# felrock/PyRacecarSimulator

Hardware: AMD Instinct MI355X
Metric: million rays/sec, 1081-beam scans (higher is better)
Workload: dtype f32

## Files before the change

pyracecarsimulator_amd/csrc/abi_fan.hip:

```cpp
#include "abi_internal.h"
#include "scan_kernels.h"
#include "crash_kernels.h"
#include "pf_kernels.h"
#include "mcl_kernels.h"
#include "launch_plan.h"

#include <array>
#include <utility>

static_assert(plan::WG == scan::WG && plan::STREAM_HDR == scan::STREAM_HDR && plan::STRIPE_BINS == scan::STRIPE_BINS &&
                  plan::STRIPE_MAX_PER_LANE == scan::STRIPE_MAX_PER_LANE && plan::DRAIN_CAP == scan::DRAIN_CAP &&
                  plan::DRAIN_FIELDS == scan::DRAIN_FIELDS && plan::INLINE_REC_BYTES == (int)sizeof(scan::BlockRec),
              "launch_plan.h and rm_kernels.h disagree about the stream kernels' LDS layout");

extern "C" int rl_method_create(rl_map *m, int kind, float max_range_px, int theta_disc,
                                rl_method **out)
{
    if (!m || !out) return fail(RL_ERR_INVALID, "rl_method_create: null pointer");
    if (!(max_range_px > 0.0f)) return fail(RL_ERR_INVALID, "max_range_px must be > 0");
    if (kind < RL_BRESENHAM || kind > RL_GIANT_LUT)
        return fail(RL_ERR_INVALID, "unknown range method kind %d", kind);
    if ((kind == RL_CDDT || kind == RL_GIANT_LUT) && (theta_disc < 2 || theta_disc > 65536))
        return fail(RL_ERR_INVALID, "theta_disc must be in [2, 65536] for CDDT / GiantLUT (got %d)",
                    theta_disc);
// ... 786 lines not shown
{
    rl_method *h = L.h;
    const int form = plan::cddt_theta_form(L.pl);
    if (form < 0) return fail(RL_ERR_INVALID, "internal: plan names an uninstantiated kernel (%s)", L.pl.name);
    const bool fused = form == plan::CDDT_THETA_FUSED;
    int rc;
    if ((rc = ensure_cddt(h, L.stream))) return rc;
    const size_t prep_bytes = (((size_t)L.n_poses * 16) + 255) & ~(size_t)255;
    if ((rc = L.cx->cddt_r.ensure(prep_bytes + (fused ? 0 : (size_t)h->cdp.theta_disc * (size_t)L.n_poses * sizeof(float)))))
        return rc;
    float4 *d_prep = (float4 *)L.cx->cddt_r.p;
    float *d_r = (float *)((char *)L.cx->cddt_r.p + prep_bytes);
    if (L.timing == 2) HIPCHK(hipEventRecord(h->ev0, L.stream));
    hipLaunchKernelGGL(cddt_theta_prep_kernel, dim3((unsigned)std::max(1, std::min((L.n_poses + 255) / 256, L.m->n_cu * 8))),
                       dim3(256), 0, L.stream, L.m->mp, L.f, h->cdp, L.d_poses, d_prep);
    if (fused) {
        hipLaunchKernelGGL(cddt_theta_fused_kernel, L.grid, L.block, L.lds, L.stream, L.m->mp, L.f, h->cdp, L.d_poses,
                           (const float4 *)d_prep, L.d_out, L.pl.nl);
        return RL_OK;
    }
    if (form == plan::CDDT_THETA_SEARCH2)
        hipLaunchKernelGGL(cddt_theta_search2_kernel, L.grid, L.block, 0, L.stream, L.m->mp, L.f, h->cdp, L.d_poses,
                           (const float4 *)d_prep, d_r, L.pl.bands);
    else
        hipLaunchKernelGGL(cddt_theta_search_kernel, L.grid, L.block, 0, L.stream, L.m->mp, L.f, h->cdp, L.d_poses,
                           (const float4 *)d_prep, d_r, L.pl.bands);
    const int n_grp = (L.n_poses + (1 << L.pl.ch) - 1) >> L.pl.ch;
    hipLaunchKernelGGL(cddt_theta_fan_kernel, dim3((unsigned)std::max(1, std::min(n_grp, L.m->n_cu * 8))), L.block, L.lds,
                       L.stream, L.m->mp, L.f, h->cdp, L.d_poses, (const float *)d_r, L.d_out, L.pl.ch, L.pl.nl);
    return RL_OK;
}

static int launch_cddt_rays(const FanLaunch &L)
{
    int rc;
    if ((rc = ensure_cddt(L.h, L.stream))) return rc;
    if (L.timing == 2) HIPCHK(hipEventRecord(L.h->ev0, L.stream));
    hipLaunchKernelGGL(cddt_fan_kernel, L.grid, L.block, 0, L.stream, L.m->mp, L.f, L.h->cdp, L.d_poses, L.d_out);
    return RL_OK;
}

static int launch_bl_stream(const FanLaunch &L)
{
    rl_method *h = L.h;
    int rc;
    if ((rc = ensure_blpad(h, L.stream))) return rc;
    if ((rc = bin_poses(h, *L.cx, L.d_poses, L.n_poses, 1, L.stream, L.pl.binning))) return rc;
    StreamParams sp{};
    sp.rec = (const PoseRec *)L.cx->rec_sorted.p;
    sp.order = (const uint32_t *)L.cx->order.p;
    sp.div_B = make_fastdiv((uint32_t)L.num_rays);
    sp.low_water = h->opt.low_water >= 0 ? h->opt.low_water : 12;
    sp.n_bands = L.pl.bands;
    sp.plain_store = L.plain_store;
    if (L.timing == 2) HIPCHK(hipEventRecord(h->ev0, L.stream));
    if (L.aux)
        hipLaunchKernelGGL((bl_fan_stream_kernel<true, 1024>), L.grid, L.block, L.lds, L.stream, L.m->mp, L.f, sp, h->blp,
                           L.d_out, L.d_hits, L.d_steps);
    else
        hipLaunchKernelGGL((bl_fan_stream_kernel<false, 1024>), L.grid, L.block, L.lds, L.stream, L.m->mp, L.f, sp, h->blp,
                           L.d_out, L.d_hits, L.d_steps);
    return RL_OK;
}

static int launch_bl_lds(const FanLaunch &L)
{
    size_t lds_bl = 0;
    BlParams bp = make_bl(L.h, L.num_rays, lds_bl);
    const bool bl = L.pl.kernel == RL_K_BL_LDS;
    if (lds_bl > 48 * 1024) {
        const void *fa = bl ? reinterpret_cast<const void *>(&bl_fan_kernel<true>)
                            : reinterpret_cast<const void *>(&occ_fan_lds_kernel<true>);
        const void *fb = bl ? reinterpret_cast<const void *>(&bl_fan_kernel<false>)
                            : reinterpret_cast<const void *>(&occ_fan_lds_kernel<false>);
        HIPCHK(hipFuncSetAttribute(fa, hipFuncAttributeMaxDynamicSharedMemorySize, (int)lds_bl));
        HIPCHK(hipFuncSetAttribute(fb, hipFuncAttributeMaxDynamicSharedMemorySize, (int)lds_bl));
    }
    if (L.timing == 2) HIPCHK(hipEventRecord(L.h->ev0, L.stream));
#define LAUNCH_BL(K) hipLaunchKernelGGL((K), L.grid, L.block, lds_bl, L.stream, L.m->mp, L.f, bp, L.d_poses, L.d_out, L.d_hits, L.d_steps)
    if (bl) { if (L.aux) LAUNCH_BL(bl_fan_kernel<true>); else LAUNCH_BL(bl_fan_kernel<false>); }
    else    { if (L.aux) LAUNCH_BL(occ_fan_lds_kernel<true>); else LAUNCH_BL(occ_fan_lds_kernel<false>); }
#undef LAUNCH_BL
    return RL_OK;
}

static int launch_rm_literal(const FanLaunch &L)
{
    const LiteralParams lt = make_literal(L.m);
    const long n_rays = (long)L.n_poses * L.num_rays;
    if (L.timing == 2) HIPCHK(hipEventRecord(L.h->ev0, L.stream));
    if (L.aux)
        hipLaunchKernelGGL((rm_literal_kernel<true, false>), L.grid, L.block, 0, L.stream, L.m->mp, L.f, lt, L.d_poses, n_rays,
                           L.d_out, L.d_hits, L.d_steps);
    else
        hipLaunchKernelGGL((rm_literal_kernel<false, false>), L.grid, L.block, 0, L.stream, L.m->mp, L.f, lt, L.d_poses, n_rays,
                           L.d_out, L.d_hits, L.d_steps);
    return RL_OK;
}

static int launch_rm_chunk(const FanLaunch &L)
{
    CrashParams cp{nullptr, 0.0, nullptr, 1};
    if (L.crash) cp = *L.crash;
    if (L.timing == 2) HIPCHK(hipEventRecord(L.h->ev0, L.stream));
#define LAUNCH_CHUNK(A, C) hipLaunchKernelGGL((rm_fan_kernel<A, C>), L.grid, L.block, L.lds, L.stream, L.m->mp, L.f, L.d_poses, \
                                              L.d_out, L.d_hits, L.d_steps, cp)
    if (L.crash) { if (L.aux) LAUNCH_CHUNK(true, true); else LAUNCH_CHUNK(false, true); }
    else         { if (L.aux) LAUNCH_CHUNK(true, false); else LAUNCH_CHUNK(false, false); }
#undef LAUNCH_CHUNK
    return RL_OK;
}

static int launch_rm_stream_family(const FanLaunch &L)
{
    rl_method *h = L.h;
    const rl_launch_plan &pl = L.pl;
    int rc;
    CrashParams cp{nullptr, 0.0, nullptr, 1};
    if (L.crash) cp = *L.crash;
    if ((rc = L.cx->rec.ensure((size_t)L.n_poses * sizeof(PoseRec)))) return rc;
    if ((rc = L.cx->order.ensure((size_t)L.n_poses * sizeof(uint32_t)))) return rc;
    if ((rc = L.cx->keys.ensure((size_t)L.n_poses * sizeof(uint32_t)))) return rc;
    if ((rc = ensure_step_map(h, L.stream))) return rc;
    if (pl.binning != RL_BIN_NONE &&
        (rc = bin_poses(h, *L.cx, L.d_poses, L.n_poses, 0, L.stream, pl.binning)))
        return rc;
    PadMap pm{};
    pm.pdt = (const float *)((const char *)h->pdt.p + h->pdt_base_off);
    pm.stride = h->pstride;
    pm.nstride = (int)h->pdt_mask;
    pm.pad = h->pad;
    pm.k4 = h->pdt_k4;
    pm.div_stride = make_fastdiv((uint32_t)h->pstride);
    pm.res = L.m->res;
    if (pl.code) {
        if (h->code_n <= 0 || pl.code_entries != h->code_n)
            return fail(RL_ERR_INVALID, "internal: code-map plan (%d entries) without a matching palette (%d)", pl.code_entries, h->code_n);
        pm.pdt = (const float *)((const char *)h->cmap.p + h->cbase_off);
        pm.stride = h->cstride;
        pm.nstride = (int)h->cmask;
        pm.k4 = h->ck4;
    }
    StreamParams sp{};
    sp.code_tab = (const float *)h->ctab.p;
    sp.code_n = pl.code ? h->code_n : 0;
    sp.tail_g1 = pl.gen1 > 0 ? pl.gen1 / std::max(pl.bands, 1) : 0;
    sp.tail_pct = std::min(h->opt.tail_pct, h->opt.tail_wg_pct);
    sp.rec = (const PoseRec *)L.cx->rec_sorted.p;
    sp.order = (const uint32_t *)L.cx->order.p;
    sp.d0 = (const float *)L.cx->d0.p;
    if ((rc = ensure_fan_table(h, L.f, L.fov, L.stream, &sp.fan_tab))) return rc;
    sp.div_B = make_fastdiv((uint32_t)L.num_rays);
    sp.low_water = h->opt.low_water >= 0 ? h->opt.low_water : ((pl.record_source != 0 && pl.slots >= 2) ? 20 : 12);
    sp.n_bands = pl.bands;
    sp.raw_poses = L.d_poses;
    sp.map = L.m->d_mp;
    sp.k_max = pl.k_max;
    sp.cpp = (uint32_t)((L.num_rays + 63) / 64);
    sp.div_cpp = make_fastdiv(sp.cpp);
    sp.drain_prio = h->drain_prio;
    sp.spec_drain = h->spec_drain;
    sp.spec_stretch = h->spec_stretch;
    sp.drain_cap = h->drain_cap;
    sp.drain_stretch = h->drain_stretch;
    sp.group_drain = h->group_drain;
    if (pl.kernel == RL_K_RM_STREAM_LIT) sp.lit = make_literal(L.m);
    sp.plain_store = L.plain_store;
    sp.dbg = nullptr;
    const int waves_per_wg = pl.block / 64;
    if (h->opt.debug_stamps) {
        if ((rc = L.cx->dbg.ensure((size_t)pl.grid * waves_per_wg * 4 * sizeof(uint64_t)))) return rc;
        sp.dbg = (unsigned long long *)L.cx->dbg.p;
        h->last_dbg = L.cx->dbg.p;
    }
    sp.stripe = pl.record_source == 2 ? 1 : pl.record_source == 3 ? 2 : 0;
    sp.run_log2 = pl.run_log2;
    h->last_grid = pl.grid * waves_per_wg / WAVES_PER_WG;
    const bool handoff = h->handoff && pl.slots >= 2 && pl.tiled && h->spec_drain > 0 && !h->opt.debug_stamps &&
                         pl.kernel == RL_K_RM_STREAM && !pl.code;
    int cap_log2 = 4;
    const int n_src = pl.grid * waves_per_wg;
    if (handoff) {
        cap_log2 = h->handoff_cap >= 64 ? 6 : (h->handoff_cap >= 32 ? 5 : (h->handoff_cap >= 16 ? 4 : 3));
        if ((rc = L.cx->left_rec.ensure(((size_t)n_src << cap_log2) * sizeof(LeftoverRec)))) return rc;
        if ((rc = L.cx->left_cnt.ensure((size_t)n_src * sizeof(uint32_t)))) return rc;
        sp.left_rec = (LeftoverRec *)L.cx->left_rec.p;
        sp.left_cnt = (uint32_t *)L.cx->left_cnt.p;
        sp.left_cap_log2 = cap_log2;
        sp.drain_cap = std::min(sp.drain_cap, 1 << cap_log2);
    }
    if (L.timing == 2) HIPCHK(hipEventRecord(h->ev0, L.stream));
    if ((rc = dispatch_rm_stream(pl, L.stream, pm, L.f, sp, L.d_out, L.d_hits, L.d_steps, cp))) return rc;
    if (handoff) {
        const int lw = h->handoff_wg / 64;
        const int n_lw = (n_src + (64 >> cap_log2) - 1) / (64 >> cap_log2);
        const dim3 lgrid((unsigned)((n_lw + lw - 1) / lw)), lblock((unsigned)h->handoff_wg);
        if (L.crash)
            hipLaunchKernelGGL((rm_leftover_kernel<true>), lgrid, lblock, 0, L.stream, pm, L.f, (const LeftoverRec *)sp.left_rec,
                               (const uint32_t *)sp.left_cnt, n_src, cap_log2, h->drain_stretch, sp.plain_store, L.d_out, cp);
        else
            hipLaunchKernelGGL((rm_leftover_kernel<false>), lgrid, lblock, 0, L.stream, pm, L.f, (const LeftoverRec *)sp.left_rec,
                               (const uint32_t *)sp.left_cnt, n_src, cap_log2, h->drain_stretch, sp.plain_store, L.d_out, cp);
    }
    return RL_OK;
}

FanCall FanCall::slice(int p0, int np, CrashParams *marks) const
{
    const size_t r0 = (size_t)p0 * num_rays;
// ... 889 lines not shown
```

pyracecarsimulator_amd/csrc/abi_internal.h:

```cpp
#pragma once
#pragma GCC visibility push(default)
#include "../../include/scanlib.h"
#pragma GCC visibility pop
#include "scan_params.h"
#include "literal_math.h"

#include <hip/hip_runtime.h>

#include <algorithm>
#include <climits>
#include <cmath>
#include <cstdarg>
#include <cstdio>
#include <cstring>
#include <atomic>
#include <condition_variable>
#include <functional>
#include <memory>
#include <mutex>
#include <shared_mutex>
#include <new>
#include <string>
#include <thread>
#include <type_traits>
// ... 141 lines not shown
        const int rc = b.ensure(n);
        return rc ? rc : up((T *)b, host, n);
    }
    template <class T>
    int fill(DevPtr<T> &b, int byte, size_t n)
    {
        const int rc = b.ensure(n);
        if (rc) return rc;
        HIPCHK(hipMemsetAsync((T *)b, byte, n * sizeof(T), st));
        return RL_OK;
    }
    template <class T>
    int zero(DevPtr<T> &b, size_t n)
    {
        return fill(b, 0, n);
    }
    template <class T>
    int down(T *host_or_null, const T *dev, size_t n)
    {
        if (host_or_null) HIPCHK(hipMemcpyAsync(host_or_null, dev, n * sizeof(T), hipMemcpyDeviceToHost, st));
        return RL_OK;
    }
    template <class T>
    int down(T *host_or_null, const DevPtr<T> &dev, size_t n)
    {
        return down(host_or_null, (const T *)dev, n);
    }
    int finish()
    {
        finished = true;
        HIPCHK(hipStreamSynchronize(st));
        return RL_OK;
    }
};

struct rl_map {
    std::vector<rl_map *> reps;
    int device = 0;
    int clock_khz = 0;
    int rows = 0, cols = 0;
    float res = 0, ox = 0, oy = 0, oyaw = 0;
    DevPtr<uint8_t> d_occ;
    DevPtr<uint8_t> d_occ_base;
    DevPtr<int32_t> d_stamp;
    Pinned<int32_t> pin_stamp;
    int stamp_cap = 0, n_stamped = 0;
    DevPtr<int> d_g;
    DevPtr<float> d_dt;
    DevPtr<uint32_t> d_bits;
    int bits_stride = 0;
    Stream stream;
    std::atomic<uint64_t> epoch{0};
    MapParams mp{};
    DevPtr<MapParams> d_mp;
    bool want_edges = false;
    DevPtr<uint32_t> d_edges, d_n_edges;
    Pinned<uint32_t> pin_n_edges;
    uint32_t n_edges = 0;
    int n_cu = 256;
    std::mutex mu;
    std::shared_mutex tables_mu;
    std::shared_mutex multi_mu;
    std::atomic<bool> broken{false};
};

struct LaunchCtx {
    hipStream_t stream = nullptr;
    bool bound = false;
    uint64_t last_use = 0;
    DevBuf rec, rec_sorted, order, keys, hist, pose_first, dbg, d0, cddt_r;
    DevBuf left_rec, left_cnt;
    DevBuf pf_r;
    int crash_epoch = 0;
};
constexpr int N_LAUNCH_CTX = 8;

struct TableDep {
    Event ev;
    hipStream_t built_on = nullptr;
    bool pending = false;
};


struct MultiPool {
    struct Worker {
        std::thread th;
        std::mutex mu;
        std::condition_variable cv;
        const std::function<int()> *job = nullptr;
        bool has = false, done = false, stop = false;
        int rc = 0;
        std::string err;
        int device = 0;
    };
    std::vector<std::unique_ptr<Worker>> w;

    void start(const std::vector<int> &devices)
    {
        for (size_t i = 1; i < devices.size(); ++i) {
            auto wk = std::make_unique<Worker>();
            wk->device = devices[i];
            Worker *raw = wk.get();
            wk->th = std::thread([raw]() {
                (void)hipSetDevice(raw->device);
                std::unique_lock<std::mutex> lk(raw->mu);
                for (;;) {
                    raw->cv.wait(lk, [raw]() { return raw->has || raw->stop; });
// ... 242 lines not shown
```

pyracecarsimulator_amd/csrc/abi_map.hip:

```cpp
#include "abi_internal.h"
#include "edt_kernels.h"

static thread_local std::string g_err = "";

int fail(int code, const char *fmt, ...)
{
    char buf[512];
    va_list ap;
    va_start(ap, fmt);
    vsnprintf(buf, sizeof buf, fmt, ap);
    va_end(ap);
    g_err = buf;
    return code;
}

int fail_map_broken() { return fail(RL_ERR_INVALID, "multi-device map is inconsistent after a failed update: destroy it"); }
const std::string &last_error() { return g_err; }
void set_last_error(const std::string &msg) { g_err = msg; }

extern "C" const char *rl_last_error(void) { return g_err.c_str(); }
extern "C" const char *rl_version(void) { return "scanlib-amd 0.6 (gfx950)"; }

extern "C" int rl_device_count(void)
{
// ... 131 lines not shown
    if (m->want_edges) m->n_edges = *m->pin_n_edges;
    return RL_OK;
}

extern "C" int rl_map_create(const uint8_t *occ, int rows, int cols, float res, float ox,
                             float oy, float oyaw, int device, rl_map **out)
{
    if (!occ || !out) return fail(RL_ERR_INVALID, "rl_map_create: null pointer");
    if (rows <= 0 || cols <= 0 || rows > 16384 || cols > 16384)
        return fail(RL_ERR_INVALID, "rl_map_create: rows/cols must be in [1,16384] (got %dx%d)",
                    rows, cols);
    if (!(res > 0.0f)) return fail(RL_ERR_INVALID, "rl_map_create: resolution must be > 0");
    int rc = check_device(device);
    if (rc) return rc;
    std::unique_ptr<rl_map, decltype(&rl_map_destroy)> own(new (std::nothrow) rl_map(), rl_map_destroy);
    rl_map *m = own.get();
    if (!m) return fail(RL_ERR_NOMEM, "out of host memory");
    m->device = device;
    m->rows = rows;
    m->cols = cols;
    m->res = res;
    m->ox = ox;
    m->oy = oy;
    m->oyaw = oyaw;
    m->bits_stride = (cols + 31) / 32;
    if (hipSetDevice(device) != hipSuccess) return fail(RL_ERR_HIP, "hipSetDevice failed");
    hipDeviceProp_t prop;
    if (hipGetDeviceProperties(&prop, device) == hipSuccess) {
        m->n_cu = prop.multiProcessorCount;
        m->clock_khz = prop.clockRate;
    }
    const size_t n = (size_t)rows * cols;
    if (m->stream.create() != hipSuccess || m->d_occ.alloc(n) || m->d_g.alloc(n * sizeof(int)) ||
        m->d_dt.alloc(n * sizeof(float)) || m->d_bits.alloc((size_t)rows * m->bits_stride * sizeof(uint32_t)))
        return fail(RL_ERR_NOMEM, "device allocation for a %dx%d map failed", rows, cols);
    if (hipMemcpyAsync(m->d_occ, occ, n, hipMemcpyHostToDevice, m->stream) != hipSuccess)
        return fail(RL_ERR_HIP, "map upload failed");
    if ((rc = map_build_tables(m))) return rc;

    MapParams &p = m->mp;
    p.dt = m->d_dt;
    p.bits = m->d_bits;
    p.bits_stride = m->bits_stride;
    p.rows = rows;
    p.cols = cols;
    p.frows = (float)rows;
    p.fcols = (float)cols;
    p.res = res;
    p.inv_res = (float)(1.0 / (double)res);
    p.ox = ox;
    p.oy = oy;
    p.wa = -oyaw;
    host_sincosf(p.wa, p.wa_sin, p.wa_cos);
    if (m->d_mp.alloc(sizeof(MapParams)) || hipMemcpy(m->d_mp, &m->mp, sizeof(MapParams), hipMemcpyHostToDevice) != hipSuccess)
        return fail(RL_ERR_NOMEM, "map parameter upload failed");
    *out = own.release();
    return RL_OK;
}

extern "C" int rl_map_create_multi(const uint8_t *occ, int rows, int cols, float res, float ox, float oy,
                                   float oyaw, const int *devices, int n_devices, rl_map **out)
{
    if (!occ || !out || !devices) return fail(RL_ERR_INVALID, "rl_map_create_multi: null pointer");
    if (n_devices < 1 || n_devices > 64) return fail(RL_ERR_INVALID, "rl_map_create_multi: 1..64 devices (got %d)", n_devices);
    std::unique_ptr<rl_map, decltype(&rl_map_destroy)> own(new (std::nothrow) rl_map(), rl_map_destroy);
    rl_map *m = own.get();
    if (!m) return fail(RL_ERR_NOMEM, "out of host memory");
    for (int i = 0; i < n_devices; ++i) {
        rl_map *r = nullptr;
        const int rc = rl_map_create(occ, rows, cols, res, ox, oy, oyaw, devices[i], &r);
        if (rc) {
            const std::string keep = g_err;
            own.reset();
            g_err = keep;
            return rc;
        }
        m->reps.push_back(r);
    }
    const rl_map *r0 = m->reps[0];
    m->device = r0->device;
    m->rows = rows;
    m->cols = cols;
    m->res = res;
    m->ox = ox;
    m->oy = oy;
    m->oyaw = oyaw;
    m->n_cu = r0->n_cu;
    m->clock_khz = r0->clock_khz;
    m->mp = r0->mp;
    *out = own.release();
    return RL_OK;
}

extern "C" int rl_map_n_devices(const rl_map *m) { return m ? (m->reps.empty() ? 1 : (int)m->reps.size()) : 0; }

extern "C" rl_map *rl_map_replica(rl_map *m, int i)
{
    if (!m) return nullptr;
    if (m->reps.empty()) return i == 0 ? m : nullptr;
    return (i >= 0 && i < (int)m->reps.size()) ? m->reps[i] : nullptr;
}

extern "C" int rl_map_update(rl_map *m, const uint8_t *occ)
{
    if (!m || !occ) return fail(RL_ERR_INVALID, "rl_map_update: null pointer");
    if (!m->reps.empty()) {
        std::lock_guard<std::mutex> lk(m->mu);
        std::unique_lock<std::shared_mutex> wl(m->multi_mu);
// ... 122 lines not shown
```

pyracecarsimulator_amd/csrc/rm_kernels.h:

```cpp
#pragma once
#include "scan_device.h"
#include "scan_params.h"
#include "literal_math.h"

namespace scan {

constexpr int WG = 256;
constexpr int WAVES_PER_WG = WG / 64;

struct CrashParams {
    const double *edge;
    double thresh;
    int *first_crashed;
    int group;
    int mark;
};

__device__ __forceinline__ void crash_note(const CrashParams &cp, uint32_t pose)
{
    if (cp.group == 0) {
        cp.first_crashed[pose] = cp.mark;
        return;
    }
    int *slot = &cp.first_crashed[pose / (uint32_t)cp.group];
// ... 173 lines not shown
    for (uint32_t i = lo; i < hi; ++i) {
        const float d = val[i];
        if (d > 0.0f) {
            idx[i] = k;
            if (k < cap) tab[k] = __builtin_fmaxf(d * coeff, 1.0f);
            ++k;
        }
    }
    if (tid == 0) {
        if (total + 2u <= cap) {
            tab[total] = PDT_HIT;
            tab[total + 1] = PDT_OUTSIDE;
        }
        n_out[0] = total + 2u;
        n_out[1] = total + 2u <= cap ? 0u : 1u;
    }
}

template <int ES>
__global__ __launch_bounds__(256) void pad_code_tiled_kernel(const float *__restrict__ dt, int rows, int cols,
                                                             void *__restrict__ cmap, TiledGeom tg, float coeff,
                                                             float max_range, const uint32_t *__restrict__ idx,
                                                             uint32_t nb, const uint32_t *__restrict__ n_pal)
{
    const uint32_t n_free = n_pal[0] - 2u;
    const int pr = blockIdx.y;
    const int r = pr - tg.padr;
    for (int pc = blockIdx.x * blockDim.x + threadIdx.x; pc < tg.pcols; pc += gridDim.x * blockDim.x) {
        const int c = pc - tg.pad;
        uint32_t code = n_free + 1u;
        if (r >= 0 && r < rows && c >= 0 && c < cols) {
            const float d = dt[(size_t)r * cols + c];
            if (d <= 0.0f) {
                code = n_free;
            } else if (__builtin_fmaxf(d * coeff, 1.0f) < max_range) {
                const uint32_t d2 = (uint32_t)__builtin_fmaf(d, d, 0.5f);
                code = d2 < nb ? idx[d2] : n_free + 1u;
            }
        }
        char *at = reinterpret_cast<char *>(cmap) + code_tiled_byte(pr, pc, tg.K, ES);
        if (ES == 1) *reinterpret_cast<uint16_t *>(at) = (uint16_t)(code << 2);
        else *reinterpret_cast<uint8_t *>(at) = (uint8_t)code;
    }
}

#define PDT_NO_RAY 2.5e38f
__device__ __forceinline__ float pose_first_step(const MapParams &m, float gx, float gy, uint32_t flags,
                                                 float coeff)
{
    if (flags & POSE_INVALID) return PDT_NO_RAY;
    const float v = m.dt[(size_t)(int)gy * m.cols + (int)gx];
    return v <= 0.0f ? 0.0f : __builtin_fmaxf(v * coeff, 1.0f);
}

__device__ __forceinline__ uint32_t tile_key(int ty, int tx, int tiles_xs, int n_tiles)
{
    const int tiles_x = tiles_xs & 0xffff, rps = tiles_xs >> 16;
    if (rps == 0) return (uint32_t)(ty * tiles_x + tx);
    const int tiles_y = n_tiles / tiles_x;
    const int y0 = (ty / rps) * rps, h = min(rps, tiles_y - y0);
    return (uint32_t)(y0 * tiles_x + tx * h + (ty - y0));
}

__device__ __forceinline__ uint32_t pose_record(const MapParams &m, const float *__restrict__ poses,
                                                int p, int tile_shift, int tiles_x, int n_tiles,
                                                PoseRec &r, bool walk_outside = false)
{
    float thg;
    world_to_grid(m, poses[3 * (size_t)p], poses[3 * (size_t)p + 1], poses[3 * (size_t)p + 2], r.gx,
                  r.gy, thg);
    det_sincosf(thg, r.st, r.ct);
    const bool fin = (r.ct - r.ct) + (r.st - r.st) == 0.0f;
    const bool inb = r.gx > -1.0f && r.gx < m.fcols && r.gy > -1.0f && r.gy < m.frows;
    if (walk_outside) {
        const bool sane = fin && __builtin_fabsf(r.gx) < 1e9f && __builtin_fabsf(r.gy) < 1e9f;
        if (!sane) {
            r.gx = 0.0f; r.gy = 0.0f; r.ct = 1.0f; r.st = 0.0f;
            return ((uint32_t)n_tiles - 1) | POSE_INVALID;
        }
        if (!inb) return (uint32_t)n_tiles - 1;
    } else if (!(fin && inb)) {
        r.gx = 0.0f; r.gy = 0.0f; r.ct = 1.0f; r.st = 0.0f;
        return ((uint32_t)n_tiles - 1) | POSE_INVALID;
    }
    return tile_key((int)r.gy >> tile_shift, (int)r.gx >> tile_shift, tiles_x, n_tiles);
}

__device__ __forceinline__ uint32_t pose_record_lit(const MapParams &m, const LiteralParams &lp, const float *__restrict__ poses,
                                                    int p, PoseRec &r)
{
    const float xw = poses[3 * (size_t)p], yw = poses[3 * (size_t)p + 1], thw = poses[3 * (size_t)p + 2];
    float x = (xw - m.ox) * m.inv_res;
    float y = (yw - m.oy) * m.inv_res;
    const float temp = x;
    x = lp.wcos * x - lp.wsin * y;
    y = lp.wsin * temp + lp.wcos * y;
    r.gx = x;
    r.gy = y;
    r.ct = thw;
    r.st = 0.0f;
    const bool fin = (thw - thw) == 0.0f;
    const bool inb = x > -1.0f && x < m.fcols && y > -1.0f && y < m.frows;
    if (!(fin && inb)) {
        r.gx = 0.0f; r.gy = 0.0f; r.ct = 0.0f;
        return POSE_INVALID;
    }
    return 0u;
}

__global__ __launch_bounds__(1024) void pose_bin_kernel(MapParams m, const float *__restrict__ poses,
                                                        int n, PoseRec *__restrict__ rec,
                                                        PoseRec *__restrict__ rec_sorted,
                                                        uint32_t *__restrict__ order,
                                                        uint32_t *__restrict__ keys, int tile_shift,
                                                        int tiles_x, int n_tiles, int do_sort, int walk_outside,
                                                        float *__restrict__ d0, float coeff)
{
    extern __shared__ uint32_t hist[];
    uint32_t *part = hist + n_tiles;
    const int tid = threadIdx.x;
    for (int i = tid; i < n_tiles; i += 1024) hist[i] = 0;
    __syncthreads();
    for (int p = tid; p < n; p += 1024) {
        PoseRec r;
        const uint32_t kf = pose_record(m, poses, p, tile_shift, tiles_x, n_tiles, r, walk_outside != 0);
        const uint32_t flag = kf & POSE_INVALID, key = kf & ~POSE_INVALID;
        if (do_sort) {
            rec[p] = r;
            keys[p] = key | flag;
            atomicAdd(&hist[key], 1u);
        } else {
            rec_sorted[p] = r;
            order[p] = (uint32_t)p | flag;
            if (d0) d0[p] = pose_first_step(m, r.gx, r.gy, flag, coeff);
        }
    }
    if (!do_sort) return;
    __syncthreads();
    const int E = (n_tiles + 1023) / 1024;
    uint32_t local = 0;
    for (int e = 0; e < E; ++e) {
        int i = tid * E + e;
        if (i < n_tiles) local += hist[i];
    }
    part[tid] = local;
    __syncthreads();
    for (int off = 1; off < 1024; off <<= 1) {
        uint32_t v = tid >= off ? part[tid - off] : 0;
        __syncthreads();
        part[tid] += v;
        __syncthreads();
    }
    uint32_t base = part[tid] - local;
    for (int e = 0; e < E; ++e) {
        int i = tid * E + e;
        if (i < n_tiles) {
            uint32_t c = hist[i];
            hist[i] = base;
            base += c;
        }
    }
    __syncthreads();
    for (int p = tid; p < n; p += 1024) {
        const uint32_t kf = keys[p];
        const uint32_t slot = atomicAdd(&hist[kf & ~POSE_INVALID], 1u);
        order[slot] = (uint32_t)p | (kf & POSE_INVALID);
        const PoseRec r = rec[p];
        rec_sorted[slot] = r;
        if (d0) d0[slot] = pose_first_step(m, r.gx, r.gy, kf, coeff);
    }
}

template <bool KEYS_ONLY>
__global__ __launch_bounds__(1024) void pose_bin_small_kernel(MapParams m, const float *__restrict__ poses,
                                                              int n, PoseRec *__restrict__ rec_sorted,
                                                              uint32_t *__restrict__ order,
                                                              int tile_shift, int tiles_x, int n_tiles,
                                                              int walk_outside, float *__restrict__ d0, float coeff)
{
    extern __shared__ uint32_t hist[];
    uint32_t *part = hist + n_tiles;
    const int tid = threadIdx.x;
    for (int i = tid; i < n_tiles; i += 1024) hist[i] = 0;
    __syncthreads();
    PoseRec r[8];
    uint32_t kf[8];
#pragma unroll
    for (int u = 0; u < 8; ++u) {
        const int p = tid + u * 1024;
        kf[u] = 0;
        if (p < n) {
            if (KEYS_ONLY) {
                float gx, gy, thg;
                world_to_grid(m, poses[3 * (size_t)p], poses[3 * (size_t)p + 1], 0.0f, gx, gy, thg);
                const bool inb = gx > -1.0f && gx < m.fcols && gy > -1.0f && gy < m.frows;
                kf[u] = inb ? tile_key((int)gy >> tile_shift, (int)gx >> tile_shift, tiles_x, n_tiles) : (uint32_t)n_tiles - 1;
            } else {
                kf[u] = pose_record(m, poses, p, tile_shift, tiles_x, n_tiles, r[u], walk_outside != 0);
            }
            atomicAdd(&hist[kf[u] & ~POSE_INVALID], 1u);
        }
    }
    __syncthreads();
    const int E = (n_tiles + 1023) / 1024;
    uint32_t local = 0;
    for (int e = 0; e < E; ++e) {
        int i = tid * E + e;
        if (i < n_tiles) local += hist[i];
    }
    uint32_t incl = local;
    const int lane = tid & 63, wave = tid >> 6;
#pragma unroll
    for (int off = 1; off < 64; off <<= 1) {
        const uint32_t o = (uint32_t)__shfl_up((int)incl, off);
        if (lane >= off) incl += o;
    }
    if (lane == 63) part[wave] = incl;
    __syncthreads();
    uint32_t wave_base = 0;
    {
        const uint32_t v = lane < 16 ? part[lane] : 0u;
        uint32_t wi = v;
#pragma unroll
        for (int off = 1; off < 16; off <<= 1) {
            const uint32_t o = (uint32_t)__shfl_up((int)wi, off);
            if (lane >= off) wi += o;
        }
        wave_base = (uint32_t)__shfl((int)(wi - v), wave);
    }
    uint32_t base = wave_base + incl - local;
    for (int e = 0; e < E; ++e) {
        int i = tid * E + e;
        if (i < n_tiles) {
            uint32_t c = hist[i];
            hist[i] = base;
            base += c;
        }
    }
    __syncthreads();
#pragma unroll
    for (int u = 0; u < 8; ++u) {
        const int p = tid + u * 1024;
        if (p < n) {
            const uint32_t slot = atomicAdd(&hist[kf[u] & ~POSE_INVALID], 1u);
            order[slot] = (uint32_t)p | (kf[u] & POSE_INVALID);
            if (!KEYS_ONLY) {
                rec_sorted[slot] = r[u];
// ... 707 lines not shown
        "s_add_u32 %[n], %[n], %[n2]\n\t"
        "s_cmp_gt_u32 %[n], %[low]\n\t"
        "s_cbranch_scc1 L_march3_%=\n\t"
        "s_mov_b64 exec, %[mA]\n\t"
        "s_waitcnt vmcnt(2)\n\t"
        "v_add_f32_e32 v20, v20, %[dA]\n\t"
        "v_cmpx_gt_f32_e32 %[mx], v20\n\t"
        "s_mov_b64 %[mA], exec\n\t"
        "s_mov_b64 exec, %[mB]\n\t"
        "s_waitcnt vmcnt(1)\n\t"
        "v_add_f32_e32 v28, v28, %[dB]\n\t"
        "v_cmpx_gt_f32_e32 %[mx], v28\n\t"
        "s_mov_b64 %[mB], exec\n\t"
        "s_mov_b64 exec, %[mC]\n\t"
        "s_waitcnt vmcnt(0)\n\t"
        "v_add_f32_e32 v36, v36, %[dC]\n\t"
        "v_cmpx_gt_f32_e32 %[mx], v36\n\t"
        "s_mov_b64 %[mC], exec\n\t"
        "s_mov_b64 exec, %[save]\n\t"
        : [tA] "+{v20}"(tA), [cA] "+v"(cA), [rA] "+v"(rA), [dA] "+v"(dA), [tB] "+{v28}"(tB), [cB] "+v"(cB),
          [rB] "+v"(rB), [dB] "+v"(dB), [tC] "+{v36}"(tC), [cC] "+v"(cC), [rC] "+v"(rC), [dC] "+v"(dC),
          [save] "=&s"(save), [mA] "=&s"(mA), [mB] "=&s"(mB), [mC] "=&s"(mC), [n] "=&s"(n), [n2] "=&s"(n2)
        : [dyA] "{v22}"(dyA), [dxA] "{v23}"(dxA), [gxA] "{v24}"(gxA), [gyA] "{v25}"(gyA), [dyB] "{v30}"(dyB),
          [dxB] "{v31}"(dxB), [gxB] "{v32}"(gxB), [gyB] "{v33}"(gyB), [dyC] "{v38}"(dyC), [dxC] "{v39}"(dxC),
          [gxC] "{v40}"(gxC), [gyC] "{v41}"(gyC), [mx] "s"(max_range), [stride] "s"(stride),
          [nstride] "s"(nstride), [k4] "v"(k4), [base] "s"(pdt), [lit] "n"(LIT ? 1 : 0), [low] "s"(low), [tiled] "n"(TILED ? 1 : 0)
        : "v26", "v27", "v34", "v35", "v42", "v43", "vcc", "scc", "memory");
}


struct PadMap {
    const float *pdt;
    int stride, nstride, pad;
    uint32_t k4;
    FastDiv div_stride;
    float res;
};

struct __attribute__((aligned(16))) LeftoverRec {
    float gx, gy, dx, dy;
    float t, d_last;
    uint32_t oidx;
    uint32_t pose;
};

struct StreamParams {
    const PoseRec *rec;
    const uint32_t *order;
    const float *d0;
    const float2 *fan_tab;
    FastDiv div_B;
    int low_water;
    int n_bands;
    const float *raw_poses;
    const MapParams *map;
    int k_max;
    uint32_t cpp;
    FastDiv div_cpp;
    int drain_prio;
    int spec_drain;
    int spec_stretch;
    int drain_cap;
    int drain_stretch;
    int group_drain;
    LiteralParams lit;
    int run_log2;
    int stripe;
    int plain_store;
    unsigned long long *dbg;
    LeftoverRec *left_rec;
    uint32_t *left_cnt;
    int left_cap_log2;
    const float *code_tab;
    int code_n;
    int tail_g1, tail_pct;
};


constexpr int STRIPE_BINS = 64;
constexpr int STRIPE_MAX_PER_LANE = 8;

__device__ __forceinline__ int stripe_row_bin(const MapParams &m, const float *__restrict__ poses, int p)
{
    float gx, gy, thg;
    world_to_grid(m, poses[3 * (size_t)p], poses[3 * (size_t)p + 1], 0.0f, gx, gy, thg);
    const float u = gy * ((float)STRIPE_BINS / m.frows);
    return u >= 0.0f ? (u < (float)STRIPE_BINS ? (int)u : STRIPE_BINS - 1) : 0;
}

__device__ __forceinline__ void wave_counts_prefix(const int *c, int nw, int lane, int wave, int &pre, int &tot)
{
    const int v = lane < nw ? c[lane] : 0;
    int incl = v;
#pragma unroll
    for (int off = 1; off < 64; off <<= 1) {
        const int o = __shfl_up(incl, off);
        if (lane >= off) incl += o;
    }
    tot = __shfl(incl, 63);
    pre = __shfl(incl - v, wave);
}

template <int NT>
__device__ __forceinline__ uint32_t stripe_band_list(const MapParams &m, const float *__restrict__ poses,
                                                     int P, uint32_t lo_rank, uint32_t hi_rank,
                                                     uint32_t *__restrict__ list, int *__restrict__ scratch)
{
    constexpr int NW = NT / 64;
// ... 31 lines not shown
    const unsigned long long below = (1ull << lane) - 1ull;
#pragma unroll 1
    for (int u = 0; u * NT < P; ++u) {
        const int p = u * NT + tid;
        const int byte = (int)((packed >> (8 * u)) & 0xffull);
        const int bin = byte == 0xff ? -1 : byte;
        const bool is_cl = bin == cl, is_ch = bin == ch && ch != cl;
        const unsigned long long b_cl = __ballot(is_cl), b_ch = __ballot(is_ch);
        if (lane == 0) wc[wave] = __popcll(b_cl) | (__popcll(b_ch) << 16);
        __syncthreads();
        int pre, tot;
        wave_counts_prefix(wc, NW, lane, wave, pre, tot);
        const int pre_cl = pre & 0xffff, pre_ch = pre >> 16, tot_cl = tot & 0xffff, tot_ch = tot >> 16;
        const int idx_cl = cnt_cl + pre_cl + __popcll(b_cl & below);
        const int idx_ch = cnt_ch + pre_ch + __popcll(b_ch & below);
        const bool member = (bin > cl && bin < ch) ||
                            (is_cl && idx_cl >= skip_lo && (cl != ch || idx_cl < take_hi)) ||
                            (is_ch && idx_ch < take_hi);
        const unsigned long long b_m = __ballot(member);
        if (lane == 0) wc[2 * NW + wave] = __popcll(b_m);
        __syncthreads();
        int pre_m, tot_m;
        wave_counts_prefix(wc + 2 * NW, NW, lane, wave, pre_m, tot_m);
        if (member) list[npos + pre_m + __popcll(b_m & below)] = (uint32_t)p;
        cnt_cl += tot_cl;
        cnt_ch += tot_ch;
        npos += (uint32_t)tot_m;
        __syncthreads();
    }
    return npos;
}

struct __attribute__((aligned(32))) BlockRec {
    float gx, gy, ct, st;
    float d0;
    uint32_t obase;
    uint32_t j0nv;
    uint32_t pose;
};

constexpr uint32_t NO_RAY = 0xffffffffu;

constexpr int DRAIN_CAP = 64;
constexpr int DRAIN_FIELDS = 7;

template <bool AUX, bool CRASH, int NT, bool INLINE, bool TILED, int SLOTS = 1, bool LIT = false, int CODE = 0>
__global__ __launch_bounds__(NT) __attribute__((amdgpu_num_sgpr(80), amdgpu_waves_per_eu(8, 8)))
void rm_fan_stream_kernel(PadMap pm, FanParams f, StreamParams sp, float *__restrict__ out,
                          int32_t *__restrict__ hits, uint16_t *__restrict__ steps, CrashParams cp)
{
    static_assert(CODE == 0 || (TILED && SLOTS == 2 && !AUX), "code map: tiled layout, two rays per lane, no diagnostics");
    static_assert(!LIT || (INLINE && TILED && !AUX), "literal stream form: INLINE records, tiled step map, no diagnostics");
    extern __shared__ __attribute__((aligned(32))) float lds_f[];
    const unsigned long long t_entry = sp.dbg ? wall_clock64() : 0ull;
    uint32_t *q_next = reinterpret_cast<uint32_t *>(lds_f);
    uint32_t *crash_seen = reinterpret_cast<uint32_t *>(lds_f + 2);
    const size_t tabw = CODE ? ((size_t)sp.code_n + 1) & ~(size_t)1 : 0;
    float2 *fan_cs = reinterpret_cast<float2 *>(lds_f + STREAM_HDR + tabw);
    double *edge_l = reinterpret_cast<double *>(lds_f + STREAM_HDR + tabw + 2 * (size_t)f.num_rays);
    const size_t tables = STREAM_HDR + tabw + (CRASH ? 4 : 2) * (size_t)f.num_rays;
    constexpr int DRAIN_F = DRAIN_FIELDS + (CRASH ? 2 : 0);
    constexpr size_t DRAIN_WORDS = (SLOTS >= 2 && TILED) ? (size_t)(NT / 64) * DRAIN_F * DRAIN_CAP : 0;
    uint32_t *drain_scr = reinterpret_cast<uint32_t *>(lds_f + ((tables + 7) & ~(size_t)7)) +
                          (size_t)(threadIdx.x >> 6) * DRAIN_F * DRAIN_CAP;
    BlockRec *lrec = reinterpret_cast<BlockRec *>(lds_f + ((tables + 7) & ~(size_t)7) + DRAIN_WORDS);
    if (threadIdx.x == 0) *q_next = 0;
    if (CRASH && threadIdx.x < STREAM_HDR - 2) crash_seen[threadIdx.x] = 0xffffffffu;
    for (int j = threadIdx.x; j < f.num_rays; j += NT) {
        fan_cs[j] = sp.fan_tab[j];
        if (CRASH) edge_l[j] = cp.edge[j];
    }
    if (CODE) {
        if ((uint32_t)(uintptr_t)lds_f != 0u) __builtin_trap();
        for (int j = threadIdx.x; j < sp.code_n; j += NT) lds_f[STREAM_HDR + j] = sp.code_tab[j];
    }

    const int nb = sp.n_bands;
    const int band = (int)(blockIdx.x % (unsigned)nb);
    const uint32_t g = blockIdx.x / (unsigned)nb;
    const uint32_t G = ((uint32_t)gridDim.x - (uint32_t)band + (uint32_t)nb - 1) / (uint32_t)nb;
    const uint32_t seg_lo = (uint32_t)(((long)f.n_poses * band) / nb);
    const uint32_t seg_hi = (uint32_t)(((long)f.n_poses * (band + 1)) / nb);
    const uint32_t seg_rays = (seg_hi - seg_lo) * (uint32_t)f.num_rays;
    const uint32_t seg_chunks = INLINE ? (seg_hi - seg_lo) * sp.cpp : (seg_rays + 63u) >> 6;
    const uint32_t rl = (uint32_t)sp.run_log2, rmask = (1u << rl) - 1u;
    const uint32_t seg_runs = (seg_chunks + rmask) >> rl;
    uint32_t own_first = g, own_stride = G, own_limit = seg_runs;
    if (sp.tail_g1 > 0 && G > (uint32_t)sp.tail_g1) {
        const uint32_t G1 = (uint32_t)sp.tail_g1, R1 = seg_runs - (seg_runs * (uint32_t)sp.tail_pct) / 100u;
        if (g < G1) {
            own_stride = G1;
            own_limit = R1;
        } else {
            own_first = R1 + (g - G1);
            own_stride = G - G1;
        }
    }
    const uint32_t K = (own_first < own_limit ? (own_limit - own_first + own_stride - 1) / own_stride : 0) << rl;
    const uint32_t total = K << 6;
    auto blkidx_of = [&](uint32_t i) { return ((own_first + (i >> rl) * own_stride) << rl) + (i & rmask); };
    auto blk_of = [&](uint32_t i) { return blkidx_of(i) << 6; };
    const unsigned lane = threadIdx.x & 63;
    if (INLINE) {
        const MapParams mp = *sp.map;
        uint32_t *list = reinterpret_cast<uint32_t *>(lrec + sp.k_max);
        if (sp.stripe == 1 && seg_hi > seg_lo)
            stripe_band_list<NT>(mp, sp.raw_poses, f.n_poses, seg_lo, seg_hi, list,
                                 reinterpret_cast<int *>(list + (seg_hi - seg_lo) + 1));
        for (uint32_t i = threadIdx.x; i < K; i += NT) {
            const uint32_t b = blkidx_of(i);
            BlockRec br{0.0f, 0.0f, 1.0f, 0.0f, PDT_NO_RAY, 0u, 0u, 0u};
            if (b < seg_chunks) {
                const uint32_t p0 = fast_div(b, sp.div_cpp);
                const uint32_t j0 = (b - p0 * sp.cpp) << 6;
                const uint32_t nvalid = min(64u, (uint32_t)f.num_rays - j0);
                const uint32_t pid = sp.stripe == 1 ? list[p0]
                                   : sp.stripe == 2 ? (sp.order[seg_lo + p0] & ~POSE_INVALID) : seg_lo + p0;
                PoseRec r;
                const uint32_t kf = LIT ? pose_record_lit(mp, sp.lit, sp.raw_poses, (int)pid, r)
                                        : pose_record(mp, sp.raw_poses, (int)pid, 0, 1, 1, r);
                br.gx = r.gx; br.gy = r.gy; br.ct = r.ct; br.st = r.st;
                br.d0 = pose_first_step(mp, r.gx, r.gy, kf, f.step_coeff);
                br.obase = (pid * (uint32_t)f.num_rays + j0) << 2;
                br.j0nv = j0 | (nvalid << 16);
                br.pose = pid;
            }
            lrec[i] = br;
        }
    }
    __syncthreads();
    const float INF = __builtin_inff();

    unsigned long long t_start = 0, t_drain = 0;
    uint32_t n_serv = 0, ns_drain = 0, drain_samples = 0;
    if (sp.dbg) t_start = wall_clock64();

    struct Slot {
        float gx, gy, dx, dy, t, d_last;
        int pc, pr;
        uint32_t oidx;
        uint32_t pose;
        int jbeam;
    };
    auto claim = [&](Slot &s, uint32_t q) -> bool {
        if (INLINE) {
            const uint4 *rp = reinterpret_cast<const uint4 *>(lrec + (q >> 6));
            const uint4 ra = rp[0], rb = rp[1];
            const uint32_t l = q & 63u;
            const bool valid = l < (rb.z >> 16);
            const uint32_t j = (rb.z & 0xffffu) + l;
            s.gx = __builtin_bit_cast(float, ra.x);
            s.gy = __builtin_bit_cast(float, ra.y);
            if (LIT) {
                const float aj = (float)j * f.inc;
                const float th = __builtin_bit_cast(float, ra.z) + (f.amin + aj);
                const float thp = -th + sp.lit.rotation_const;
                s.dy = lit_cosf(thp);
                s.dx = lit_sinf(thp);
            } else {
                const float2 cs = fan_cs[j];
                const float ct = __builtin_bit_cast(float, ra.z), st = __builtin_bit_cast(float, ra.w);
                s.dx = __builtin_fmaf(ct, cs.x, -(st * cs.y));
                s.dy = __builtin_fmaf(st, cs.x, ct * cs.y);
            }
            s.oidx = valid ? rb.y + (l << 2) : NO_RAY;
            if (CRASH) {
                s.pose = rb.w;
                s.jbeam = (int)j;
            }
            s.d_last = __builtin_bit_cast(float, rb.x);
            s.t = valid ? s.d_last : __builtin_inff();
            return valid;
        }
        const uint32_t ray = blk_of(q >> 6) + (q & 63);
        if (ray >= seg_rays) return false;
        const uint32_t spose = fast_div(ray, sp.div_B);
        const int j = (int)(ray - spose * (uint32_t)f.num_rays);
        const uint32_t si = seg_lo + spose;
        const uint32_t po = *reinterpret_cast<const uint32_t *>(reinterpret_cast<const char *>(sp.order) + (si << 2));
        const PoseRec pr_ = *reinterpret_cast<const PoseRec *>(reinterpret_cast<const char *>(sp.rec) + (si << 4));
// ... 365 lines not shown
```

Measured before the change: 193,500.

## Overlap stream-kernel prologue loads and pass map params by value

Reworks the stream kernel prologue so fan-table, edge, palette and first-round pose loads are issued into registers before their LDS stores. This lets the global load latencies overlap instead of serializing. MapParams is now passed in the kernel argument struct rather than through a device pointer, which removes a dependent load and the per-map device allocation. Band division uses a precomputed fast divider, and the first-step distance-table load is hoisted ahead of the validity check. The kernel argument block grows, and the first-step cell load is now issued speculatively even for invalid poses.

```diff
diff --git a/pyracecarsimulator_amd/csrc/abi_fan.hip b/pyracecarsimulator_amd/csrc/abi_fan.hip
--- a/pyracecarsimulator_amd/csrc/abi_fan.hip
+++ b/pyracecarsimulator_amd/csrc/abi_fan.hip
@@ -862,6 +862,7 @@
     sp.div_B = make_fastdiv((uint32_t)L.num_rays);
     sp.low_water = h->opt.low_water >= 0 ? h->opt.low_water : 12;
     sp.n_bands = L.pl.bands;
+    sp.div_bands = make_fastdiv((uint32_t)L.pl.bands);
     sp.plain_store = L.plain_store;
     if (L.timing == 2) HIPCHK(hipEventRecord(h->ev0, L.stream));
     if (L.aux)
@@ -963,8 +964,9 @@
     sp.div_B = make_fastdiv((uint32_t)L.num_rays);
     sp.low_water = h->opt.low_water >= 0 ? h->opt.low_water : ((pl.record_source != 0 && pl.slots >= 2) ? 20 : 12);
     sp.n_bands = pl.bands;
+    sp.div_bands = make_fastdiv((uint32_t)pl.bands);
     sp.raw_poses = L.d_poses;
-    sp.map = L.m->d_mp;
+    sp.map = L.m->mp;
     sp.k_max = pl.k_max;
     sp.cpp = (uint32_t)((L.num_rays + 63) / 64);
     sp.div_cpp = make_fastdiv(sp.cpp);
diff --git a/pyracecarsimulator_amd/csrc/abi_internal.h b/pyracecarsimulator_amd/csrc/abi_internal.h
--- a/pyracecarsimulator_amd/csrc/abi_internal.h
+++ b/pyracecarsimulator_amd/csrc/abi_internal.h
@@ -217,7 +217,6 @@
     Stream stream;
     std::atomic<uint64_t> epoch{0};
     MapParams mp{};
-    DevPtr<MapParams> d_mp;
     bool want_edges = false;
     DevPtr<uint32_t> d_edges, d_n_edges;
     Pinned<uint32_t> pin_n_edges;
diff --git a/pyracecarsimulator_amd/csrc/abi_map.hip b/pyracecarsimulator_amd/csrc/abi_map.hip
--- a/pyracecarsimulator_amd/csrc/abi_map.hip
+++ b/pyracecarsimulator_amd/csrc/abi_map.hip
@@ -207,8 +207,6 @@
     p.oy = oy;
     p.wa = -oyaw;
     host_sincosf(p.wa, p.wa_sin, p.wa_cos);
-    if (m->d_mp.alloc(sizeof(MapParams)) || hipMemcpy(m->d_mp, &m->mp, sizeof(MapParams), hipMemcpyHostToDevice) != hipSuccess)
-        return fail(RL_ERR_NOMEM, "map parameter upload failed");
     *out = own.release();
     return RL_OK;
 }
diff --git a/pyracecarsimulator_amd/csrc/rm_kernels.h b/pyracecarsimulator_amd/csrc/rm_kernels.h
--- a/pyracecarsimulator_amd/csrc/rm_kernels.h
+++ b/pyracecarsimulator_amd/csrc/rm_kernels.h
@@ -249,6 +249,12 @@
     const float v = m.dt[(size_t)(int)gy * m.cols + (int)gx];
     return v <= 0.0f ? 0.0f : __builtin_fmaxf(v * coeff, 1.0f);
 }
+__device__ __forceinline__ float pose_first_step_at(const MapParams &m, size_t cell0, uint32_t flags, float coeff)
+{
+    const float v = m.dt[cell0];
+    if (flags & POSE_INVALID) return PDT_NO_RAY;
+    return v <= 0.0f ? 0.0f : __builtin_fmaxf(v * coeff, 1.0f);
+}
 
 __device__ __forceinline__ uint32_t tile_key(int ty, int tx, int tiles_xs, int n_tiles)
 {
@@ -259,16 +265,16 @@
     return (uint32_t)(y0 * tiles_x + tx * h + (ty - y0));
 }
 
-__device__ __forceinline__ uint32_t pose_record(const MapParams &m, const float *__restrict__ poses,
-                                                int p, int tile_shift, int tiles_x, int n_tiles,
-                                                PoseRec &r, bool walk_outside = false)
+__device__ __forceinline__ uint32_t pose_record_of(const MapParams &m, float xw, float yw, float thw,
+                                                   int tile_shift, int tiles_x, int n_tiles,
+                                                   PoseRec &r, size_t &cell0, bool walk_outside = false)
 {
     float thg;
-    world_to_grid(m, poses[3 * (size_t)p], poses[3 * (size_t)p + 1], poses[3 * (size_t)p + 2], r.gx,
-                  r.gy, thg);
+    world_to_grid(m, xw, yw, thw, r.gx, r.gy, thg);
+    const bool inb = r.gx > -1.0f && r.gx < m.fcols && r.gy > -1.0f && r.gy < m.frows;
+    cell0 = inb ? (size_t)(int)r.gy * m.cols + (int)r.gx : 0;
     det_sincosf(thg, r.st, r.ct);
     const bool fin = (r.ct - r.ct) + (r.st - r.st) == 0.0f;
-    const bool inb = r.gx > -1.0f && r.gx < m.fcols && r.gy > -1.0f && r.gy < m.frows;
     if (walk_outside) {
         const bool sane = fin && __builtin_fabsf(r.gx) < 1e9f && __builtin_fabsf(r.gy) < 1e9f;
         if (!sane) {
@@ -283,10 +289,18 @@
     return tile_key((int)r.gy >> tile_shift, (int)r.gx >> tile_shift, tiles_x, n_tiles);
 }
 
-__device__ __forceinline__ uint32_t pose_record_lit(const MapParams &m, const LiteralParams &lp, const float *__restrict__ poses,
-                                                    int p, PoseRec &r)
-{
-    const float xw = poses[3 * (size_t)p], yw = poses[3 * (size_t)p + 1], thw = poses[3 * (size_t)p + 2];
+__device__ __forceinline__ uint32_t pose_record(const MapParams &m, const float *__restrict__ poses,
+                                                int p, int tile_shift, int tiles_x, int n_tiles,
+                                                PoseRec &r, bool walk_outside = false)
+{
+    size_t cell0;
+    return pose_record_of(m, poses[3 * (size_t)p], poses[3 * (size_t)p + 1], poses[3 * (size_t)p + 2], tile_shift,
+                          tiles_x, n_tiles, r, cell0, walk_outside);
+}
+
+__device__ __forceinline__ uint32_t pose_record_lit(const MapParams &m, const LiteralParams &lp, float xw, float yw,
+                                                    float thw, PoseRec &r, size_t &cell0)
+{
     float x = (xw - m.ox) * m.inv_res;
     float y = (yw - m.oy) * m.inv_res;
     const float temp = x;
@@ -298,6 +312,7 @@
     r.st = 0.0f;
     const bool fin = (thw - thw) == 0.0f;
     const bool inb = x > -1.0f && x < m.fcols && y > -1.0f && y < m.frows;
+    cell0 = inb ? (size_t)(int)y * m.cols + (int)x : 0;
     if (!(fin && inb)) {
         r.gx = 0.0f; r.gy = 0.0f; r.ct = 0.0f;
         return POSE_INVALID;
@@ -378,6 +393,18 @@
     extern __shared__ uint32_t hist[];
     uint32_t *part = hist + n_tiles;
     const int tid = threadIdx.x;
+    float px[8], py[8];
+    if (KEYS_ONLY) {
+#pragma unroll
+        for (int u = 0; u < 8; ++u) {
+            px[u] = py[u] = 0.0f;
+            if (u * 1024 < n) {
+                const size_t pc = (size_t)min(tid + u * 1024, n - 1);
+                px[u] = poses[3 * pc];
+                py[u] = poses[3 * pc + 1];
+            }
+        }
+    }
     for (int i = tid; i < n_tiles; i += 1024) hist[i] = 0;
     __syncthreads();
     PoseRec r[8];
@@ -389,7 +416,7 @@
         if (p < n) {
             if (KEYS_ONLY) {
                 float gx, gy, thg;
-                world_to_grid(m, poses[3 * (size_t)p], poses[3 * (size_t)p + 1], 0.0f, gx, gy, thg);
+                world_to_grid(m, px[u], py[u], 0.0f, gx, gy, thg);
                 const bool inb = gx > -1.0f && gx < m.fcols && gy > -1.0f && gy < m.frows;
                 kf[u] = inb ? tile_key((int)gy >> tile_shift, (int)gx >> tile_shift, tiles_x, n_tiles) : (uint32_t)n_tiles - 1;
             } else {
@@ -1203,8 +1230,9 @@
     FastDiv div_B;
     int low_water;
     int n_bands;
+    FastDiv div_bands;
     const float *raw_poses;
-    const MapParams *map;
+    MapParams map;
     int k_max;
     uint32_t cpp;
     FastDiv div_cpp;
@@ -1342,6 +1370,7 @@
     static_assert(CODE == 0 || (TILED && SLOTS == 2 && !AUX), "code map: tiled layout, two rays per lane, no diagnostics");
     static_assert(!LIT || (INLINE && TILED && !AUX), "literal stream form: INLINE records, tiled step map, no diagnostics");
     extern __shared__ __attribute__((aligned(32))) float lds_f[];
+    asm volatile("" ::"s"(sp.cpp), "s"(gridDim.x));
     const unsigned long long t_entry = sp.dbg ? wall_clock64() : 0ull;
     uint32_t *q_next = reinterpret_cast<uint32_t *>(lds_f);
     uint32_t *crash_seen = reinterpret_cast<uint32_t *>(lds_f + 2);
@@ -1356,21 +1385,28 @@
     BlockRec *lrec = reinterpret_cast<BlockRec *>(lds_f + ((tables + 7) & ~(size_t)7) + DRAIN_WORDS);
     if (threadIdx.x == 0) *q_next = 0;
     if (CRASH && threadIdx.x < STREAM_HDR - 2) crash_seen[threadIdx.x] = 0xffffffffu;
-    for (int j = threadIdx.x; j < f.num_rays; j += NT) {
-        fan_cs[j] = sp.fan_tab[j];
-        if (CRASH) edge_l[j] = cp.edge[j];
-    }
-    if (CODE) {
-        if ((uint32_t)(uintptr_t)lds_f != 0u) __builtin_trap();
-        for (int j = threadIdx.x; j < sp.code_n; j += NT) lds_f[STREAM_HDR + j] = sp.code_tab[j];
-    }
-
-    const int nb = sp.n_bands;
-    const int band = (int)(blockIdx.x % (unsigned)nb);
-    const uint32_t g = blockIdx.x / (unsigned)nb;
-    const uint32_t G = ((uint32_t)gridDim.x - (uint32_t)band + (uint32_t)nb - 1) / (uint32_t)nb;
-    const uint32_t seg_lo = (uint32_t)(((long)f.n_poses * band) / nb);
-    const uint32_t seg_hi = (uint32_t)(((long)f.n_poses * (band + 1)) / nb);
+    const uint32_t tid = threadIdx.x;
+    constexpr int PRO_TAB = 2;
+    float2 t_cs[PRO_TAB];
+    double t_edge[PRO_TAB];
+#pragma unroll
+    for (int u = 0; u < PRO_TAB; ++u) {
+        const uint32_t j = min(tid + (uint32_t)(u * NT), (uint32_t)f.num_rays - 1u);
+        t_cs[u] = sp.fan_tab[j];
+        if (CRASH) t_edge[u] = cp.edge[j];
+    }
+    float t_pal = 0.0f;
+    if (CODE) t_pal = sp.code_tab[min(tid, (uint32_t)sp.code_n - 1u)];
+    const uint32_t nb = (uint32_t)sp.n_bands;
+    const uint32_t g = fast_div(blockIdx.x, sp.div_bands);
+    const uint32_t band = blockIdx.x - g * nb;
+    const uint32_t G = fast_div((uint32_t)gridDim.x - band + nb - 1u, sp.div_bands);
+    auto band_cut = [&](uint32_t b) -> uint32_t {
+        const unsigned long long pb = (unsigned long long)(uint32_t)f.n_poses * b;
+        return (pb >> 32) ? (uint32_t)(pb / nb) : fast_div((uint32_t)pb, sp.div_bands);
+    };
+    const uint32_t seg_lo = band_cut(band);
+    const uint32_t seg_hi = band_cut(band + 1u);
     const uint32_t seg_rays = (seg_hi - seg_lo) * (uint32_t)f.num_rays;
     const uint32_t seg_chunks = INLINE ? (seg_hi - seg_lo) * sp.cpp : (seg_rays + 63u) >> 6;
     const uint32_t rl = (uint32_t)sp.run_log2, rmask = (1u << rl) - 1u;
@@ -1391,31 +1427,81 @@
     auto blkidx_of = [&](uint32_t i) { return ((own_first + (i >> rl) * own_stride) << rl) + (i & rmask); };
     auto blk_of = [&](uint32_t i) { return blkidx_of(i) << 6; };
     const unsigned lane = threadIdx.x & 63;
+    const MapParams &mp = sp.map;
+    uint32_t *list = reinterpret_cast<uint32_t *>(lrec + sp.k_max);
+    if (INLINE && sp.stripe == 1 && seg_hi > seg_lo)
+        stripe_band_list<NT>(mp, sp.raw_poses, f.n_poses, seg_lo, seg_hi, list,
+                             reinterpret_cast<int *>(list + (seg_hi - seg_lo) + 1));
+    auto blk_pose = [&](uint32_t i, uint32_t &p0, uint32_t &j0) -> bool {
+        const uint32_t b = blkidx_of(i);
+        const bool own = i < K && b < seg_chunks;
+        p0 = own ? fast_div(b, sp.div_cpp) : 0u;
+        j0 = own ? (b - p0 * sp.cpp) << 6 : 0u;
+        return own;
+    };
+    auto blk_pid = [&](bool own, uint32_t p0) -> uint32_t {
+        if (sp.stripe == 1) return own ? list[p0] : 0u;
+        if (sp.stripe == 2) return sp.order[own ? seg_lo + p0 : 0u] & ~POSE_INVALID;
+        return own ? seg_lo + p0 : 0u;
+    };
+    auto blk_rec = [&](bool own, uint32_t j0, uint32_t pid, float xw, float yw, float thw) -> BlockRec {
+        BlockRec br{0.0f, 0.0f, 1.0f, 0.0f, PDT_NO_RAY, 0u, 0u, 0u};
+        PoseRec r;
+        size_t cell0;
+        const uint32_t kf = LIT ? pose_record_lit(mp, sp.lit, xw, yw, thw, r, cell0)
+                                : pose_record_of(mp, xw, yw, thw, 0, 1, 1, r, cell0);
+        const float d0 = pose_first_step_at(mp, cell0, kf, f.step_coeff);
+        if (own) {
+            const uint32_t nvalid = min(64u, (uint32_t)f.num_rays - j0);
+            br.gx = r.gx; br.gy = r.gy; br.ct = r.ct; br.st = r.st;
+            br.d0 = d0;
+            br.obase = (pid * (uint32_t)f.num_rays + j0) << 2;
+            br.j0nv = j0 | (nvalid << 16);
+            br.pose = pid;
+        }
+        return br;
+    };
+    const bool wave_recs = INLINE && (uint32_t)__builtin_amdgcn_readfirstlane((int)(tid & ~63u)) < K;
+    bool own = false;
+    uint32_t p0 = 0u, j0 = 0u, pid = 0u;
+    if (wave_recs) {
+        own = blk_pose(tid, p0, j0);
+        pid = blk_pid(own, p0);
+    }
+    float xw = 0.0f, yw = 0.0f, thw = 0.0f;
+    if (wave_recs) {
+        const float *pp = sp.raw_poses + 3 * (size_t)pid;
+        xw = pp[0]; yw = pp[1]; thw = pp[2];
+    }
+#pragma unroll
+    for (int u = 0; u < PRO_TAB; ++u) {
+        const uint32_t j = tid + (uint32_t)(u * NT);
+        if (j < (uint32_t)f.num_rays) {
+            fan_cs[j] = t_cs[u];
+            if (CRASH) edge_l[j] = t_edge[u];
+        }
+    }
+#pragma unroll 1
+    for (int j = (int)tid + PRO_TAB * NT; j < f.num_rays; j += NT) {
+        fan_cs[j] = sp.fan_tab[j];
+        if (CRASH) edge_l[j] = cp.edge[j];
+    }
+    if (CODE) {
+        if ((uint32_t)(uintptr_t)lds_f != 0u) __builtin_trap();
+        if (tid < (uint32_t)sp.code_n) lds_f[STREAM_HDR + tid] = t_pal;
+#pragma unroll 1
+        for (int j = (int)tid + NT; j < sp.code_n; j += NT) lds_f[STREAM_HDR + j] = sp.code_tab[j];
+    }
+    if (wave_recs) {
+        const BlockRec br = blk_rec(own, j0, pid, xw, yw, thw);
+        if (tid < K) lrec[tid] = br;
+    }
     if (INLINE) {
-        const MapParams mp = *sp.map;
-        uint32_t *list = reinterpret_cast<uint32_t *>(lrec + sp.k_max);
-        if (sp.stripe == 1 && seg_hi > seg_lo)
-            stripe_band_list<NT>(mp, sp.raw_poses, f.n_poses, seg_lo, seg_hi, list,
-                                 reinterpret_cast<int *>(list + (seg_hi - seg_lo) + 1));
-        for (uint32_t i = threadIdx.x; i < K; i += NT) {
-            const uint32_t b = blkidx_of(i);
-            BlockRec br{0.0f, 0.0f, 1.0f, 0.0f, PDT_NO_RAY, 0u, 0u, 0u};
-            if (b < seg_chunks) {
-                const uint32_t p0 = fast_div(b, sp.div_cpp);
-                const uint32_t j0 = (b - p0 * sp.cpp) << 6;
-                const uint32_t nvalid = min(64u, (uint32_t)f.num_rays - j0);
-                const uint32_t pid = sp.stripe == 1 ? list[p0]
-                                   : sp.stripe == 2 ? (sp.order[seg_lo + p0] & ~POSE_INVALID) : seg_lo + p0;
-                PoseRec r;
-                const uint32_t kf = LIT ? pose_record_lit(mp, sp.lit, sp.raw_poses, (int)pid, r)
-                                        : pose_record(mp, sp.raw_poses, (int)pid, 0, 1, 1, r);
-                br.gx = r.gx; br.gy = r.gy; br.ct = r.ct; br.st = r.st;
-                br.d0 = pose_first_step(mp, r.gx, r.gy, kf, f.step_coeff);
-                br.obase = (pid * (uint32_t)f.num_rays + j0) << 2;
-                br.j0nv = j0 | (nvalid << 16);
-                br.pose = pid;
-            }
-            lrec[i] = br;
+        for (uint32_t i = tid + NT; i < K; i += NT) {
+            own = blk_pose(i, p0, j0);
+            pid = blk_pid(own, p0);
+            const float *pp = sp.raw_poses + 3 * (size_t)pid;
+            lrec[i] = blk_rec(own, j0, pid, pp[0], pp[1], pp[2]);
         }
     }
     __syncthreads();
```

New measurement: 196,100 (median of 6 runs). +1.3%, better.
